# zhengchen1999/DOVE

Measured on AMD Instinct MI355X. Metric: SR frames/s (33x720x1280 4x one-step, whole job), higher is better.
Workload: dtype bf16; 1 GPU; synthetic 33x720x1280 HR clip (LR 180x320, 4x), one-step t=399, CogVideoX1.5-5B VAE + 42-layer DiT random-init, 1 clip per GPU (BASELINE configs[1]); weight_sums=True, vae_streams=2, variant=headline (bf16)

## Files before the change

### dove_amd/csrc/elementwise.hip

```cpp
#include "common.h"
#include "../../include/dove_hip.h"

__device__ __forceinline__ float load_any(const void* p, long long i, int dt) {
  return dt == DOVE_F32 ? ((const float*)p)[i] : bf2f(((const bf16_t*)p)[i]);
}
__device__ __forceinline__ void store_any(void* p, long long i, int dt, float v) {
  if (dt == DOVE_F32) ((float*)p)[i] = v;
  else ((bf16_t*)p)[i] = f2bf(v);
}

__global__ void cl_from_ncthw_kernel(const void* __restrict__ x, int dt, int C, long long npix, int Cp,
                                     float scale, float shift, bf16_t* __restrict__ y) {
  const long long p = (long long)blockIdx.x * blockDim.x + threadIdx.x;
  if (p >= npix) return;
  bf16_t* yr = y + p * Cp;
  for (int c0 = 0; c0 < Cp; c0 += 8) {
    float f[8];
#pragma unroll
    for (int e = 0; e < 8; ++e) {
      const int c = c0 + e;
      f[e] = c < C ? load_any(x, (long long)c * npix + p, dt) * scale + shift : 0.f;
    }
    *(uint4*)(yr + c0) = pack8(f);
  }
}

extern "C" int dove_cl_from_ncthw(const void* x, int dtype, int C, long long npix, int Cp, float scale, float shift,
                                   void* y, void* stream) {
  DOVE_CHECK_ARG(x && y, "cl_from_ncthw: null pointer");
  DOVE_CHECK_ARG(dtype == DOVE_F32 || dtype == DOVE_BF16, "cl_from_ncthw: bad dtype %d", dtype);
  DOVE_CHECK_ARG(Cp % 8 == 0 && Cp >= C && C > 0 && npix > 0, "cl_from_ncthw: need Cp %% 8 == 0, Cp >= C");
  hipLaunchKernelGGL(cl_from_ncthw_kernel, dim3((unsigned)((npix + 255) / 256)), dim3(256), 0, (hipStream_t)stream, x,
                     dtype, C, npix, Cp, scale, shift, (bf16_t*)y);
  DOVE_CHECK_LAUNCH("dove_cl_from_ncthw");
  return DOVE_OK;
}

__global__ void cl_im2col3x3_kernel(const void* __restrict__ x, int dt, int C, int T, int H, int W, int Cp, float scale, float shift,
                                    bf16_t* __restrict__ y) {
  const long long npix = (long long)T * H * W;
  const long long p = (long long)blockIdx.x * blockDim.x + threadIdx.x;
  if (p >= npix) return;
  const int w = (int)(p % W), h = (int)((p / W) % H);
  bf16_t* yr = y + p * Cp;
  for (int c0 = 0; c0 < Cp; c0 += 8) {
    float f[8];
#pragma unroll
    for (int e = 0; e < 8; ++e) {
      const int k = c0 + e, tap = k / C, c = k - tap * C;
      const int dy = tap / 3 - 1, dx = tap % 3 - 1;
      const bool in = tap < 9 && h + dy >= 0 && h + dy < H && w + dx >= 0 && w + dx < W;
      f[e] = in ? load_any(x, (long long)c * npix + p + (long long)dy * W + dx, dt) * scale + shift : 0.f;
    }
    *(uint4*)(yr + c0) = pack8(f);
  }
}
extern "C" int dove_cl_im2col3x3_from_ncthw(const void* x, int dtype, int C, int T, int H, int W, int Cp, float scale, float shift, void* y,
                                            void* stream) {
  DOVE_CHECK_ARG(x && y, "cl_im2col3x3: null pointer");
  DOVE_CHECK_ARG(dtype == DOVE_F32 || dtype == DOVE_BF16, "cl_im2col3x3: bad dtype %d", dtype);
  DOVE_CHECK_ARG(C > 0 && Cp % 8 == 0 && Cp >= 9 * C && T > 0 && H > 0 && W > 0, "cl_im2col3x3: need Cp %% 8 == 0 and Cp >= 9 C");
  const long long npix = (long long)T * H * W;
  hipLaunchKernelGGL(cl_im2col3x3_kernel, dim3((unsigned)((npix + 255) / 256)), dim3(256), 0, (hipStream_t)stream, x, dtype, C, T, H, W, Cp,
                     scale, shift, (bf16_t*)y);
  DOVE_CHECK_LAUNCH("dove_cl_im2col3x3_from_ncthw");
  return DOVE_OK;
}

__global__ void ncthw_from_cl_kernel(const bf16_t* __restrict__ x, long long ld, int C, long long npix, float scale,
                                     float shift, float lo, float hi, void* __restrict__ y, int dt) {
  const long long p = (long long)blockIdx.x * blockDim.x + threadIdx.x;
  if (p >= npix) return;
  const bf16_t* xr = x + p * ld;
  for (int c0 = 0; c0 < C; c0 += 4) {
    const uint2 v = *(const uint2*)(xr + c0);
    const float f[4] = {__uint_as_float(v.x << 16), __uint_as_float(v.x & 0xffff0000u), __uint_as_float(v.y << 16),
                        __uint_as_float(v.y & 0xffff0000u)};
#pragma unroll
    for (int e = 0; e < 4; ++e)
      if (c0 + e < C) store_any(y, (long long)(c0 + e) * npix + p, dt, fminf(fmaxf(f[e] * scale + shift, lo), hi));
  }
}

extern "C" int dove_ncthw_from_cl(const void* x, long long ld, int C, long long npix, float scale, float shift,
                                   float lo, float hi, void* y, int dtype, void* stream) {
  DOVE_CHECK_ARG(x && y, "ncthw_from_cl: null pointer");
  DOVE_CHECK_ARG(dtype == DOVE_F32 || dtype == DOVE_BF16, "ncthw_from_cl: bad dtype %d", dtype);
  DOVE_CHECK_ARG(ld % 4 == 0 && ld >= ((C + 3) / 4) * 4 && C > 0 && npix > 0, "ncthw_from_cl: ld must be a multiple of 4 covering C");
  hipLaunchKernelGGL(ncthw_from_cl_kernel, dim3((unsigned)((npix + 255) / 256)), dim3(256), 0, (hipStream_t)stream,
                     (const bf16_t*)x, ld, C, npix, scale, shift, lo, hi, y, dtype);
  DOVE_CHECK_LAUNCH("dove_ncthw_from_cl");
  return DOVE_OK;
}

__global__ __launch_bounds__(256) void conv_out_gather_kernel(const float* __restrict__ p, int ldp, int T, int H, int W, int C,
                                                              const float* __restrict__ bias, float scale, float shift, float lo, float hi,
                                                              void* __restrict__ y, int dt, int ldy) {
  extern __shared__ __attribute__((aligned(16))) float tile[];
  constexpr int TH = 8, TW = 64, RW = TW + 2, NREC = (TH + 2) * RW;
  const int lrec = ldp + 1, f4n = ldp >> 2;
  const int x0 = blockIdx.x * TW, y0 = blockIdx.y * TH, t = blockIdx.z;
  for (int i = threadIdx.x; i < NREC * f4n; i += 256) {
    const int rec = i / f4n, f4 = i - rec * f4n;
    const int ry = rec / RW, rx = rec - ry * RW;
    const int iy = y0 + ry - 1, ix = x0 + rx - 1;
    f32x4 v = {0.f, 0.f, 0.f, 0.f};
    if (iy >= 0 && iy < H && ix >= 0 && ix < W) v = *(const f32x4*)(p + (((long long)t * H + iy) * W + ix) * ldp + f4 * 4);
    float* d = tile + rec * lrec + f4 * 4;
    d[0] = v[0]; d[1] = v[1]; d[2] = v[2]; d[3] = v[3];
  }
  __syncthreads();
  const int lx = threadIdx.x & 63;
  const long long npix = (long long)T * H * W;
#pragma unroll
  for (int h2 = 0; h2 < 2; ++h2) {
    const int rr = (threadIdx.x >> 6) + 4 * h2;
// ... 354 lines not shown
```

### dove_amd/csrc/igemm.hip

```cpp
#include "igemm_args.h"


template <int BN, int BK>
struct FastCfg {
  static constexpr int BM = 128;
  static constexpr int CPR = BK / 8;
  static constexpr int CPR_LOG = (BK == 64) ? 3 : 2;
  static constexpr int RPG = 256 / CPR;
  static constexpr int NA = BM / RPG;
  static constexpr int B_SLOTS = BN * CPR;
  static constexpr int NB = (B_SLOTS + 255) / 256;
  static constexpr int A_BYTES = BM * BK * 2, B_BYTES = BN * BK * 2, STAGE = A_BYTES + B_BYTES;
  static constexpr int WN = (BN >= 128) ? 2 : 1, WM = 4 / WN;
  static constexpr int PT = (BM / WM) / 32, CT = (BN / WN) / 32;
  static constexpr int KK = BK / 16;
};

template <int BN, int BK>
__global__ __launch_bounds__(256) void igemm_fast_kernel(const IgemmArgs a) {
  using Cf = FastCfg<BN, BK>;
  constexpr int NA = Cf::NA, NB = Cf::NB, PT = Cf::PT, CT = Cf::CT, KK = Cf::KK, STAGE = Cf::STAGE, A_BYTES = Cf::A_BYTES;
  extern __shared__ __attribute__((aligned(16))) char smem[];
  const int tid = threadIdx.x, lane = tid & 63;
  const int wave = __builtin_amdgcn_readfirstlane(tid >> 6);
// ... 1023 lines not shown
namespace smallk { constexpr int ROWS = 32; }
__global__ __launch_bounds__(256) void smallk_kernel(const bf16_t* __restrict__ x, const bf16_t* __restrict__ w, const float* __restrict__ bias,
                                                     bf16_t* __restrict__ out, long long M, int cout_store, long long ldo) {
  typedef __bf16 v2bf __attribute__((ext_vector_type(2)));
  __shared__ uint4 xs[4 * smallk::ROWS][4];
  const int lane = threadIdx.x & 63, wave = threadIdx.x >> 6;
  const long long rb = (long long)blockIdx.x * 4 * smallk::ROWS;
#pragma unroll
  for (int i = 0; i < 2; ++i) {
    const int idx = threadIdx.x + i * 256;
    const long long m = rb + (idx >> 2);
    xs[idx >> 2][idx & 3] = m < M ? *(const uint4*)(x + m * 32 + (idx & 3) * 8) : uint4{0u, 0u, 0u, 0u};
  }
  const int n0 = (blockIdx.y * 64 + lane) * 4;
  const bool live = n0 < cout_store;
  uint32_t wr[4][16];
  float b[4] = {0.f, 0.f, 0.f, 0.f};
  if (live) {
#pragma unroll
    for (int j = 0; j < 4; ++j)
#pragma unroll
      for (int q = 0; q < 4; ++q) {
        const uint4 v = *(const uint4*)(w + (long long)(n0 + j) * 32 + q * 8);
        wr[j][q * 4 + 0] = v.x; wr[j][q * 4 + 1] = v.y; wr[j][q * 4 + 2] = v.z; wr[j][q * 4 + 3] = v.w;
      }
    if (bias) { b[0] = bias[n0]; b[1] = bias[n0 + 1]; b[2] = bias[n0 + 2]; b[3] = bias[n0 + 3]; }
  }
  __syncthreads();
  if (!live) return;
  const long long r0 = rb + wave * smallk::ROWS;
#pragma unroll 4
  for (int r = 0; r < smallk::ROWS; ++r) {
    const long long m = r0 + r;
    if (m >= M) break;
    uint32_t xr[16];
#pragma unroll
    for (int q = 0; q < 4; ++q) {
      const uint4 v = xs[wave * smallk::ROWS + r][q];
      xr[q * 4 + 0] = v.x; xr[q * 4 + 1] = v.y; xr[q * 4 + 2] = v.z; xr[q * 4 + 3] = v.w;
    }
    float acc[4] = {b[0], b[1], b[2], b[3]};
#pragma unroll
    for (int k = 0; k < 16; ++k)
#pragma unroll
      for (int j = 0; j < 4; ++j)
        acc[j] = __builtin_amdgcn_fdot2_f32_bf16(__builtin_bit_cast(v2bf, wr[j][k]), __builtin_bit_cast(v2bf, xr[k]), acc[j], false);
    uint2 o;
    o.x = pack_bf2(acc[0], acc[1]);
    o.y = pack_bf2(acc[2], acc[3]);
    *(uint2*)(out + m * ldo + n0) = o;
  }
}

enum ConvKernel { K_IGEMM = 0, K_IGEMM_FAST, K_HALO4X, K_HALO4X_UP, K_GEMM8P, K_SMALLK, K_HALO4X_SUB };
static const char* const kKernelNames[] = {"igemm_kernel", "igemm_fast_kernel", "conv3x3_halo4x_kernel", "conv3x3_halo4x_kernel", "gemm8p_kernel",
                                           "smallk_kernel", "conv3x3_halo4x_kernel"};

static inline int desc_nb(const dove_conv_desc* d) { return d->nb > 1 ? d->nb : 1; }

static ConvKernel select_kernel(const dove_conv_desc* d) {
  const long long M = (long long)desc_nb(d) * d->t_out * d->h_out * d->w_out;
  const bool frame_fits = (long long)d->h_in * d->w_in * d->cin * 2 < (1ll << 31);
  const bool plain_gemm = d->kt == 1 && d->kh == 1 && d->kw == 1 && d->stride == 1 && d->up == 0 && d->tmode == 0 &&
                          d->t_in == d->t_out && d->h_in == d->h_out && d->w_in == d->w_out && d->cout_pad % 128 == 0 && M >= 4096 &&
                          (long long)512 * d->cin * 2 < (1ll << 31);
  const bool pointwise = d->kt == 1 && d->kh == 1 && d->kw == 1 && d->stride == 1 && d->up == 0 && d->tmode == 0 && d->t_in == d->t_out &&
                         d->h_in == d->h_out && d->w_in == d->w_out;
  if (pointwise && d->cin == 32 && d->act == 0 && !d->resid && !d->gate && d->cout_store >= 128) return K_SMALLK;
  if (plain_gemm) {
    if (d->cout_pad % 256 == 0 && d->cout_store % 256 == 0 && d->cin % 128 == 0 && d->cin >= 256 && (long long)256 * d->cin * 2 < (1ll << 31) &&
        d->ldo < (1 << 20) && d->ldr < (1 << 20) && (d->act == 0 || d->act == 1))
      return K_GEMM8P;
  }
  const bool conv3 = d->kh == 3 && d->kw == 3 && d->stride == 1 && d->pad_h == 1 && d->pad_w == 1 && d->act == 0 && !d->gate &&
                     d->cout_pad % 128 == 0 && frame_fits;
  if (conv3) {
    const bool same = d->up == 0 && d->tmode == 0 && d->h_out == d->h_in && d->w_out == d->w_in && d->w_out >= 16 && d->h_out >= 16;
    const bool ups = d->up == 1 && d->kt == 1 && d->h_out == 2 * d->h_in && d->w_out == 2 * d->w_in && d->h_out >= 16 && d->w_out >= 32;
    const bool h4 = d->cout_store % 128 == 0 && d->cin % 64 == 0 && d->ldo < (1 << 20) && (!d->resid || d->ldr < (1 << 20));
    if (same && h4) return K_HALO4X;
    if (ups && h4 && d->w_sub && d->h_in >= 16 && d->w_in >= 32) return K_HALO4X_SUB;
    if (ups && h4) return K_HALO4X_UP;
  }
  const int BN = (d->cout_pad % 128 == 0) ? 128 : ((d->cout_pad % 64 == 0) ? 64 : 32);
  const bool fits = frame_fits && (long long)BN * d->cin * 2 < (1ll << 31);
  return (d->up == 0 && fits) ? K_IGEMM_FAST : K_IGEMM;
}

static bool desc_size_ok(const dove_conv_desc* d, const char* who) {
  if (d && d->struct_size == sizeof(dove_conv_desc) && d->reserved == 0) return true;
  if (d) dove_set_error("%s: dove_conv_desc.struct_size is %u, this library (ABI %d) expects %zu - the caller's binding was written "
                        "against another include/dove_hip.h", who, d->struct_size, DOVE_ABI_VERSION, sizeof(dove_conv_desc));
  else dove_set_error("%s: null descriptor", who);
  return false;
}
extern "C" const char* dove_conv_kernel_name(const dove_conv_desc* d) { return desc_size_ok(d, "conv_kernel_name") ? kKernelNames[select_kernel(d)] : ""; }

template <int BN, int BK>
static int launch_igemm_fast(const IgemmArgs& a, unsigned grid, hipStream_t s) {
  constexpr int lds = 2 * (128 * BK * 2 + BN * BK * 2);
  static PerDeviceOnce attr_set;
  if (auto once_ = attr_set.guard()) (void)hipFuncSetAttribute((const void*)igemm_fast_kernel<BN, BK>, hipFuncAttributeMaxDynamicSharedMemorySize, lds);
  hipLaunchKernelGGL((igemm_fast_kernel<BN, BK>), dim3(grid), dim3(256), lds, s, a);
  DOVE_CHECK_LAUNCH("dove_conv_igemm_bf16");
  return DOVE_OK;
}

static int cu_count() {
  static std::atomic<int> cus[DOVE_MAX_DEVICES] = {};
  int dev = 0;
  (void)hipGetDevice(&dev);
  int n = (dev >= 0 && dev < DOVE_MAX_DEVICES) ? cus[dev].load(std::memory_order_relaxed) : 0;
  if (!n) {
    n = 256;
    (void)hipDeviceGetAttribute(&n, hipDeviceAttributeMultiprocessorCount, dev);
    if (dev >= 0 && dev < DOVE_MAX_DEVICES) cus[dev].store(n, std::memory_order_relaxed);
  }
  return n;
}

extern "C" long long dove_conv_gn_partial_rows(const dove_conv_desc* d) {
  if (!desc_size_ok(d, "conv_gn_partial_rows")) return 0;
  const ConvKernel k = select_kernel(d);
  if (k != K_HALO4X && k != K_HALO4X_UP && k != K_HALO4X_SUB) return 0;
  if (d->cout_store != 128 && d->cout_store != 256 && d->cout_store != 512) return 0;
  if (d->cout_store != d->cout_pad) return 0;
  if (k == K_HALO4X_SUB) {
    const long long th = (d->h_in + halo8::TH - 1) / halo8::TH, tw = (d->w_in + halo8::TW - 1) / halo8::TW;
    return (long long)desc_nb(d) * d->t_out * th * tw * 16;
  }
  const long long th = (d->h_out + halo8::TH - 1) / halo8::TH, tw = (d->w_out + halo8::TW - 1) / halo8::TW;
  return (long long)desc_nb(d) * d->t_out * th * tw * 4;
}

static bool halo4x_plan(const dove_conv_desc* d) {
  const int tiles_w = (d->w_out + halo8::TW - 1) / halo8::TW, tiles_h = (d->h_out + halo8::TH - 1) / halo8::TH;
  const int wrem = d->w_out % halo8::TW;
  if (wrem < 1 || wrem > halo8::TW / 2) return false;
  const int cus = cu_count();
  const long long per = (long long)desc_nb(d) * d->t_out * (d->cout_pad / 128);
  auto rounds = [&](long long tiles) { return (tiles * per + cus - 1) / cus; };
  return rounds((long long)tiles_h * (tiles_w - 1)) + rounds((d->h_out + 31) / 32) < rounds((long long)tiles_h * tiles_w);
}
extern "C" int dove_conv_partial_launches(const dove_conv_desc* d) {
  if (!desc_size_ok(d, "conv_partial_launches") || select_kernel(d) != K_HALO4X) return 0;
  return halo4x_plan(d) ? 1 : 0;
}

static int conv_dispatch(const dove_conv_desc* d, void* stream, ConvKernel kern);

static bool gemm_tail_split(const dove_conv_desc* d, long long* rows_main) {
  const long long M = (long long)d->t_out * d->h_out * d->w_out;
  if (d->t_out != 1 || d->h_out != 1 || desc_nb(d) > 1) return false;
  const int cus = cu_count(), tiles_n = d->cout_pad / 256;
  const long long row_tiles = (M + gemm4x::BM - 1) / gemm4x::BM, ntiles = row_tiles * tiles_n;
  if (ntiles <= cus || ntiles % cus == 0) return false;
  const long long main_rt = (ntiles / cus) * cus / tiles_n;
// ... 110 lines not shown
      a.tiles_n = 4 * (d->cout_pad / 128);
      a.nty = a.tiles_h; a.ntx = a.tiles_w; a.h_lim = d->h_out; a.w_lim = d->w_out;
      const long long g4 = (long long)a.T_out * a.tiles_h * a.tiles_w * a.tiles_n;
      DOVE_CHECK_ARG(g4 > 0 && g4 < (1ll << 31), "conv_igemm: grid too large");
      static PerDeviceOnce attrs;
      if (auto once_ = attrs.guard()) (void)hipFuncSetAttribute((const void*)(conv3x3_halo4x_kernel<false, true>), hipFuncAttributeMaxDynamicSharedMemorySize, Halo4xCfg::LDS_BYTES);
      const int cus = cu_count();
      const unsigned grid = g4 > cus ? (unsigned)cus : (unsigned)g4;
      hipLaunchKernelGGL((conv3x3_halo4x_kernel<false, true>), dim3(grid), dim3(256), Halo4xCfg::LDS_BYTES, s, a);
      DOVE_CHECK_LAUNCH("dove_conv_igemm_bf16(halo4x sub-pixel)");
      return DOVE_OK;
    }
    case K_HALO4X:
    case K_HALO4X_UP: {
      a.gn_partial = d->gn_partial;
      a.w_first = (kern == K_HALO4X && d->kt == 3 && !d->cache) ? (const bf16_t*)d->w_first : nullptr;
      if (kern == K_HALO4X && d->kt == 3 && d->tdup) { a.tdup = d->tdup; a.w_pair = (const bf16_t*)d->w_pair; }
      a.cpg_log = d->cout_store == 128 ? 2 : (d->cout_store == 256 ? 3 : 4);
      a.tiles_w = (d->w_out + halo8::TW - 1) / halo8::TW;
      a.tiles_h = (d->h_out + halo8::TH - 1) / halo8::TH;
      a.tiles_n = d->cout_pad / 128;
      a.ty0 = a.tx0 = 0; a.nty = a.tiles_h; a.ntx = a.tiles_w; a.h_lim = d->h_out; a.w_lim = d->w_out;
      const long long g4 = (long long)a.T_out * a.tiles_h * a.tiles_w * a.tiles_n;
      DOVE_CHECK_ARG(g4 > 0 && g4 < (1ll << 31), "conv_igemm: grid too large");
      static PerDeviceOnce attr4;
      if (auto once_ = attr4.guard()) {
        (void)hipFuncSetAttribute((const void*)(conv3x3_halo4x_kernel<false>), hipFuncAttributeMaxDynamicSharedMemorySize, Halo4xCfg::LDS_BYTES);
        (void)hipFuncSetAttribute((const void*)(conv3x3_halo4x_kernel<false, false, 1>), hipFuncAttributeMaxDynamicSharedMemorySize, H4Geo<1>::LDS_BYTES);
        (void)hipFuncSetAttribute((const void*)(conv3x3_halo4x_kernel<true>), hipFuncAttributeMaxDynamicSharedMemorySize, Halo4xCfg::LDS_BYTES);
      }
      const int cus = cu_count();
      const unsigned grid = g4 > cus ? (unsigned)cus : (unsigned)g4;
      if (kern == K_HALO4X_UP) hipLaunchKernelGGL((conv3x3_halo4x_kernel<true>), dim3(grid), dim3(256), Halo4xCfg::LDS_BYTES, s, a);
      else {
        const bool wpart = halo4x_plan(d);
        const int wm = wpart ? (a.tiles_w - 1) * halo8::TW : d->w_out, cols_main = wpart ? a.tiles_w - 1 : a.tiles_w;
        auto launch = [&](int part, int nty, int tx0, int ntx, int w_lim) {
          if (nty <= 0 || ntx <= 0) return;
          IgemmArgs b = a;
          b.ty0 = 0; b.nty = nty; b.tx0 = tx0; b.ntx = ntx; b.h_lim = d->h_out; b.w_lim = w_lim;
          const long long g = (long long)b.T_out * nty * ntx * b.tiles_n;
          const unsigned gr = g > cus ? (unsigned)cus : (unsigned)g;
          if (part == 0) hipLaunchKernelGGL((conv3x3_halo4x_kernel<false, false, 0>), dim3(gr), dim3(256), H4Geo<0>::LDS_BYTES, s, b);
          else hipLaunchKernelGGL((conv3x3_halo4x_kernel<false, false, 1>), dim3(gr), dim3(256), H4Geo<1>::LDS_BYTES, s, b);
        };
        launch(0, a.tiles_h, 0, cols_main, wm);
        if (wpart) launch(1, (d->h_out + 31) / 32, cols_main, 1, d->w_out);
      }
      DOVE_CHECK_LAUNCH("dove_conv_igemm_bf16(halo4x)");
      return DOVE_OK;
    }
    default: break;
  }
  int twl = 7;
  if (d->h_out > 1) {
    twl = 4;
    if (d->w_out <= 8) twl = 3;
    if (d->w_out <= 4) twl = 2;
  }
  a.tw_log2 = twl;
  const int TW = 1 << twl, TH = 128 >> twl;
  a.tiles_w = (d->w_out + TW - 1) / TW;
  a.tiles_h = (d->h_out + TH - 1) / TH;
  const int BN = (d->cout_pad % 128 == 0) ? 128 : ((d->cout_pad % 64 == 0) ? 64 : 32);
  a.tiles_n = d->cout_pad / BN;
  const long long grid = (long long)a.T_out * a.tiles_h * a.tiles_w * a.tiles_n;
  DOVE_CHECK_ARG(grid > 0 && grid < (1ll << 31), "conv_igemm: grid too large");
  const bool fast = kern == K_IGEMM_FAST;
  const bool bk64 = (d->cin % 64 == 0);
  if (!fast) return launch_igemm_legacy(a, (unsigned)grid, BN, bk64, s);
  if (BN == 128) return bk64 ? launch_igemm_fast<128, 64>(a, (unsigned)grid, s) : launch_igemm_fast<128, 32>(a, (unsigned)grid, s);
  if (BN == 64) return bk64 ? launch_igemm_fast<64, 64>(a, (unsigned)grid, s) : launch_igemm_fast<64, 32>(a, (unsigned)grid, s);
  return bk64 ? launch_igemm_fast<32, 64>(a, (unsigned)grid, s) : launch_igemm_fast<32, 32>(a, (unsigned)grid, s);
}
```

### dove_amd/lib.py

```python
from __future__ import annotations

import ctypes as C
import os

import torch

_HERE = os.path.dirname(os.path.abspath(__file__))
LIB_PATH = os.path.join(_HERE, "libdove_hip.so")
_lib = None

F32, BF16, U8 = 0, 1, 2
METRIC_PSNR, METRIC_SSIM, METRIC_RGB_TO_Y = 1, 2, 4
COLORFIX_WAVELET, COLORFIX_ADAIN, COLORFIX_CLAMP = 1, 2, 1
YUV_444, YUV_422, YUV_420, YUV_MONO = 0, 1, 2, 3
YUV_SITING_LEFT, YUV_SITING_CENTRE = 0, 1
VIDEO_RGB_U8, VIDEO_YUV = 0, 1
RESIZE_BILINEAR, RESIZE_BICUBIC, RESIZE_AREA = 0, 1, 2
ACT_NONE, ACT_RELU, ACT_SIGMOID, ACT_TANH = 0, 1, 2, 3


class ConvDesc(C.Structure):
    _fields_ = [
        ("struct_size", C.c_uint), ("reserved", C.c_uint),
        ("x", C.c_void_p), ("cache", C.c_void_p), ("w", C.c_void_p), ("bias", C.c_void_p),
# ... 147 lines not shown
    "dove_linear_mxfp8": [_VP, _VP, _VP, _VP, _VP, _VP, _VP, _VP, _LL, _I, _I, _LL, _LL, _LL, _I, _VP],
    "dove_fr_metrics": [C.POINTER(ImageView), C.POINTER(ImageView), _I, _I, _I, _I, _I, _VP, C.c_size_t, _VP, _VP],
    "dove_color_fix": [C.POINTER(ImageView), _F, _F, C.POINTER(ImageView), _F, _F, _I, _I, _I, _I, _I, C.POINTER(ImageView), _VP,
                       C.c_size_t, _VP],
    "dove_rgb_to_yuv_u8": [C.POINTER(ImageView), _I, _I, _I, C.POINTER(YuvFormat), _VP, _VP],
    "dove_yuv_to_rgb_u8": [_VP, _I, _I, _I, C.POINTER(YuvFormat), _VP, _VP],
    "dove_plan_padding": [_I, _I, _I, _PI, _PI, _PI],
    "dove_plan_output_size": [_I, _I, _I, _PI, _PI],
    "dove_plan_temporal_chunks": [_I, _I, _I, _PI, _I],
    "dove_plan_spatial_tiles": [_I, _I, _I, _I, _I, _I, _PI, _I],
    "dove_plan_valid_region": [_PI, _I, _I, _I, _I, _I, _I, _PI, _PI],
    "dove_plan_pieces": [_I, _I, _I, _I, _I, _I, _I, _I, _I, _PI, _PI, _PI, _I],
    "dove_plan_check_coverage": [_PI, _I, _I, _I, _I],
    "dove_chunk_planner_create": [_I, _I, C.POINTER(_VP)],
    "dove_chunk_planner_next": [_VP, _LL, _I, _PLL, _PLL, _PI],
    "dove_philox_u32": [_VP, _LL, _ULL, _ULL, _ULL, _VP],
    "dove_randn": [_VP, _I, _LL, _ULL, _ULL, _ULL, _VP],
    "dove_blur2d_f32": [_VP, _I, _I, _I, _VP, _I, _I, _VP, _VP],
    "dove_resize_f32": [_VP, _I, _I, _I, _I, _I, _I, _VP, _VP],
    "dove_add_gaussian_noise_f32": [_VP, _I, _I, _I, C.POINTER(C.c_float), _I, _ULL, _ULL, _LL, _VP, _VP],
    "dove_add_poisson_noise_f32": [_VP, _I, _I, _I, C.POINTER(C.c_float), _I, _ULL, _ULL, _LL, _VP, C.c_size_t, _VP, _VP],
    "dove_jpeg_roundtrip": [_VP, _I, _I, _I, _PI, _VP, C.c_size_t, _VP, _VP],
    "dove_stitch": [_VP, _I, _I, _I, _PI, _VP, _I, _I, _I, _I, _I, _I, _VP],
    "dove_video_open": [_VP, C.POINTER(VideoParams), C.POINTER(_VP)],
    "dove_video_info": [_VP, C.POINTER(C.c_size_t), C.POINTER(C.c_size_t), _PI, _PI, _PI],
    "dove_video_push": [_VP, _VP, _I, _VP],
    "dove_video_end_of_input": [_VP],
    "dove_video_need": [_VP, _PLL, _PI],
    "dove_video_step": [_VP, _VP, C.c_size_t, _PI, _PI, _VP],
    "dove_conv2d_f32": [C.POINTER(Conv2dF32Args), _VP],
    "dove_instance_norm_f32": [_VP, _I, _I, _I, _I, _VP, _I, _F, _VP, C.c_size_t, _VP, _VP],
    "dove_corr_volume_f32": [_VP, _VP, _I, _I, _I, _I, _F, _VP, _VP],
    "dove_avgpool2_f32": [_VP, _LL, _I, _I, _VP, _VP],
    "dove_corr_lookup_f32": [_VP, _VP, _VP, _VP, _VP, _LL, _I, _I, _I, _I, _VP, _VP],
    "dove_gru_gate_f32": [_VP, _LL, _VP, _LL, _I, _I, _LL, _VP, _VP],
    "dove_gru_update_f32": [_VP, _LL, _VP, _LL, _VP, _LL, _I, _LL, _VP],
    "dove_add_f32": [_VP, _LL, _VP, _LL, _VP, _LL, _I, _LL, _I, _VP],
    "dove_convex_upsample_f32": [_VP, _LL, _VP, _I, _I, _I, _VP, _VP],
    "dove_flow_warp_error": [_VP, _VP, _I, _VP, _VP, _I, _I, _I, _VP, C.c_size_t, _VP, _VP, _VP, _VP],
    "dove_convnet_conv_f32": [C.POINTER(ConvnetConvF32Args), _VP],
    "dove_percep_prep_f32": [C.POINTER(ImageView), _I, _I, _I, _I, _F, _F, C.POINTER(C.c_float), C.POINTER(C.c_float), _VP, _VP],
    "dove_maxpool_f32": [_VP, _LL, _I, _I, _I, _I, _I, _I, _VP, _LL, _VP],
    "dove_l2pool_f32": [_VP, _LL, _I, _I, _I, _I, _VP, _LL, _VP],
    "dove_lpips_layer": [_VP, _VP, _LL, _VP, _I, _I, _I, _I, _VP, C.c_size_t, _VP, _VP],
    "dove_dists_layer": [_VP, _VP, _LL, _VP, _VP, _I, _I, _I, _I, _VP, C.c_size_t, _VP, _VP],
    "dove_niqe_features": [C.POINTER(ImageView), _I, _I, _I, _I, _VP, C.c_size_t, _VP, _VP, _VP],
    "dove_niqe_stats": [_VP, _I, _I, _VP, _VP, _VP, _VP],
    "dove_niqe_distance": [_VP, _VP, _VP, _VP, _VP],
}
PLAIN = {"dove_last_error": (C.c_char_p, []), "dove_abi_version": (C.c_int, []), "dove_comm_destroy": (None, [C.c_void_p]),
         "dove_conv_gn_partial_rows": (C.c_longlong, [C.POINTER(ConvDesc)]),
         "dove_conv_kernel_name": (C.c_char_p, [C.POINTER(ConvDesc)]),
         "dove_conv_partial_launches": (C.c_int, [C.POINTER(ConvDesc)]),
         "dove_attention_head_paths": (C.c_int, [C.POINTER(C.c_float), _I, C.POINTER(C.c_int)]),
         "dove_attention_path_name": (C.c_char_p, [_I]),
         "dove_device_info": (C.c_int, [_I, C.c_char_p, _I, C.POINTER(C.c_int), C.POINTER(C.c_longlong)]),
         "dove_destroy": (None, [_VP]),
         "dove_vae_decode_num_frames": (C.c_int, [_VP, _I]),
         "dove_get_option": (C.c_longlong, [_VP, _I]),
         "dove_comm_useful_ranks": (C.c_int, [_VP, _I, _I]),
         "dove_workspace_bytes": (C.c_size_t, [_VP, _I, _I, _I]),
         "dove_workspace_high_water": (C.c_size_t, [_VP]),
         "dove_fr_metrics_workspace_bytes": (C.c_size_t, [_I, _I, _I]),
         "dove_color_fix_workspace_bytes": (C.c_size_t, [_I, _I, _I, _I]),
         "dove_yuv_frame_bytes": (C.c_size_t, [_I, _I, _I]),
         "dove_poisson_noise_workspace_bytes": (C.c_size_t, [_I]),
         "dove_jpeg_roundtrip_workspace_bytes": (C.c_size_t, [_I, _I, _I]),
         "dove_chunk_planner_need": (C.c_longlong, [_VP]),
         "dove_chunk_planner_destroy": (None, [_VP]),
         "dove_video_workspace_bytes": (C.c_size_t, [_VP, C.POINTER(VideoParams)]),
         "dove_video_close": (None, [_VP]),
         "dove_instance_norm_f32_workspace_bytes": (C.c_size_t, [_I, _I, _I, _I]),
         "dove_flow_warp_error_workspace_bytes": (C.c_size_t, [_I, _I, _I]),
         "dove_convnet_conv_f32_kernel_name": (C.c_char_p, [C.POINTER(ConvnetConvF32Args)]),
         "dove_lpips_layer_workspace_bytes": (C.c_size_t, [_I, _I, _I]),
         "dove_dists_layer_workspace_bytes": (C.c_size_t, [_I, _I, _I, _I]),
         "dove_niqe_workspace_bytes": (C.c_size_t, [_I, _I, _I])}


def kernel_source_sha256() -> str:
    import glob
    import hashlib
    h = hashlib.sha256()
    files = sorted(glob.glob(os.path.join(_HERE, "csrc", "*.hip")) + glob.glob(os.path.join(_HERE, "csrc", "*.h")))
    files.append(os.path.join(os.path.dirname(_HERE), "include", "dove_hip.h"))
    for fn in files:
        h.update(os.path.basename(fn).encode() + b"\0")
        with open(fn, "rb") as f:
            h.update(f.read())
        h.update(b"\0")
    return h.hexdigest()


def load():
    global _lib
    if _lib is not None:
        return _lib
    if not os.path.exists(LIB_PATH):
        raise RuntimeError(f"{LIB_PATH} not found: build it with `python -c 'import __graft_entry__ as g; g.build()'` "
                           "(dove_amd has no CPU fallback)")
    lib = C.CDLL(LIB_PATH)
    for name, argt in SIGNATURES.items():
        fn = getattr(lib, name)
        fn.argtypes = argt
        fn.restype = C.c_int
    for name, (res, argt) in PLAIN.items():
# ... 42 lines not shown
```

### include/dove_hip.h

```cpp
#ifndef DOVE_HIP_H
#define DOVE_HIP_H

#include <stddef.h>

#ifdef __cplusplus
extern "C" {
#endif

#define DOVE_ABI_VERSION 15

#define DOVE_F32 0
#define DOVE_BF16 1

const char* dove_last_error(void);
int dove_abi_version(void);
int dove_device_info(int dev, char* name, int name_len, int* cu_count, long long* total_mem);

typedef struct dove_conv_desc {
  unsigned int struct_size;
  unsigned int reserved;
  const void* x;
  const void* cache;
  const void* w;
  const float* bias;
  const void* resid;
  const float* gate;
  void* out;
  int t_in, h_in, w_in, cin;
  int t_out, h_out, w_out, cout_pad, cout_store;
  int kt, kh, kw, stride, pad_h, pad_w, up, tmode, act;
  long long ldo, ldr, gate_split;
  float* gn_partial;
  int out_f32;
  int nb;
  long long cache_stride;
  const void* w_first;
  const void* w_sub;
  const void* w_pair;
  int tdup;
  int reserved2;
} dove_conv_desc;
int dove_conv_igemm_bf16(const dove_conv_desc* d, void* stream);
const char* dove_conv_kernel_name(const dove_conv_desc* d);
int dove_conv_partial_launches(const dove_conv_desc* d);
long long dove_conv_gn_partial_rows(const dove_conv_desc* d);
int dove_groupnorm_finalize_partials(const float* partial, long long rows, double count, float eps, void* ws, float* stats,
                                     void* stream);

int dove_groupnorm_stats_bf16(const void* x, long long npix, long long frame_pix, int C, float eps, void* partial_ws, int ws_blocks,
                              float* stats, void* stream);
int dove_groupnorm_sums_bf16(const void* x, long long npix, long long frame_pix, int C, void* partial_ws, int ws_blocks, double* sums,
                             void* stream);
int dove_groupnorm_finalize_sums(const double* sums, double count, float eps, float* stats, void* stream);
int dove_groupnorm_sums_from_partials(const float* partial, long long rows, void* ws, double* sums, void* stream);
int dove_groupnorm_apply_bf16(const void* x, void* y, int T, int H, int W, int C, const float* stats,
                              const float* gamma, const float* beta, int silu, const void* yb, int hz, int wz,
                              int sshift, const int* tmap, void* stream);

int dove_groupnorm_stats_nb_bf16(const void* x, int nb, long long npix, long long frame_pix, int C, float eps, void* partial_ws,
                                 int ws_blocks, float* stats, void* stream);
int dove_groupnorm_finalize_partials_nb(const float* partial, long long rows, int nb, double count, float eps, void* ws, size_t ws_bytes,
                                        float* stats, void* stream);
int dove_groupnorm_apply_nb_bf16(const void* x, void* y, int nb, int T, int H, int W, int C, const float* stats, const float* gamma,
                                 const float* beta, int silu, const void* yb, int Tz, int hz, int wz, int sshift, const int* tmap,
                                 void* stream);
int dove_avgpool_time_nb_bf16(const void* x, int nb, int T, long long frame_elems, void* y, void* stream);

int dove_layernorm_modulate_bf16(const void* x, void* y, long long rows, int D, float eps, const float* gamma,
                                 const float* beta, const float* mod, long long split, void* stream);

int dove_qkv_post_bf16(const void* qkv, long long N, long long Npad, int heads, int head_dim, int text_len,
                       const float* gq, const float* bq, const float* gk, const float* bk, const float* cosT,
                       const float* sinT, float qscale, float eps, void* Qh, void* Kh, void* Vt, int v_order, float* norm2, void* stream);
int dove_vt_quad_swap_bf16(void* Vt, long long rows, long long Npad, void* stream);
int dove_ulysses_place_bf16(const void* rq, const void* rk, const void* rv, const long long* counts, int world, int hloc, long long N,
                            long long Npad, void* Qh, void* Kh, void* Vt, float* norm2_out, void* stream);

int dove_attention_fwd_bf16(const void* Qh, const void* Kh, const void* Vt, void* O, long long N, long long Npad,
                            int heads, int head_dim, long long ldo, float* norm2, void* stream);
int dove_attention_head_paths(const float* norm2_host, int heads, int* path);
const char* dove_attention_path_name(int path);

int dove_cl_from_ncthw(const void* x, int dtype, int C, long long npix, int Cp, float scale, float shift, void* y,
                       void* stream);
int dove_ncthw_from_cl(const void* x, long long ld, int C, long long npix, float scale, float shift, float lo,
                       float hi, void* y, int dtype, void* stream);
int dove_cl_im2col3x3_from_ncthw(const void* x, int dtype, int C, int T, int H, int W, int Cp, float scale, float shift, void* y,
                                 void* stream);
int dove_conv_out_gather(const float* p, long long ldp, int T, int H, int W, int C, const float* bias, float scale, float shift, float lo,
                         float hi, void* y, int dtype, void* stream);
int dove_avgpool_time_bf16(const void* x, int T, long long frame_elems, void* y, void* stream);
int dove_posterior_sample(const void* moments, long long ld, int latent_channels, long long npix, const void* noise,
                          int noise_dtype, void* out, int out_dtype, void* stream);
int dove_axpby(const void* x, const void* y, void* out, int dtype, long long n, float a, float b, void* stream);
int dove_patchify(const void* x, int dtype, int T, int C, int H, int W, int pt, int p, void* tokens, long long ld,
                  void* stream);
int dove_unpatchify(const void* tokens, long long ld, int T, int C, int H, int W, int pt, int p, void* y, int dtype,
// ... 255 lines not shown
```

Measured before the change: 35.54 frames/s.

## Add persistent thin-K pointwise conv kernel with LDS-resident weights

Adds a persistent igemm_thin kernel for pointwise convs with small K (64–384) and narrow Cout (32/128/256). It keeps all weights resident in LDS and streams activation tiles through a per-wave ring with counted vmcnt waits, then writes output through an LDS epilogue with buffer stores. The aim is to avoid reloading weights for every tile and the poor tile shapes of the generic fast igemm on these thin GEMMs. Separately, the 3x3 im2col kernel now uses one thread per 8-channel chunk instead of one per pixel, with 32-bit index math when it fits, giving more parallelism and cheaper addressing. The price is a much larger, more complex kernel with a grid limited to one block per CU, and correctness depends on the hand-counted waits.

```diff
diff --git a/dove_amd/csrc/elementwise.hip b/dove_amd/csrc/elementwise.hip
--- a/dove_amd/csrc/elementwise.hip
+++ b/dove_amd/csrc/elementwise.hip
@@ -36,32 +36,41 @@
   return DOVE_OK;
 }
 
+template <typename I>
+__device__ __forceinline__ void cl_im2col3x3_chunk(const void* __restrict__ x, int dt, int C, I npix, int H, int W, int Cp, float scale, float shift,
+                                                   bf16_t* __restrict__ y, I i) {
+  const I cpp = (I)(Cp >> 3);
+  const I p = i / cpp;
+  if (p >= npix) return;
+  const int c0 = (int)(i - p * cpp) << 3;
+  const I row = p / (I)W;
+  const int w = (int)(p - row * (I)W), h = (int)(row % (I)H);
+  int tap = c0 / C, c = c0 - tap * C;
+  float f[8];
+#pragma unroll
+  for (int e = 0; e < 8; ++e) {
+    const int ty = tap / 3, dy = ty - 1, dx = tap - ty * 3 - 1;
+    const bool in = tap < 9 && h + dy >= 0 && h + dy < H && w + dx >= 0 && w + dx < W;
+    f[e] = in ? load_any(x, (long long)c * (long long)npix + (long long)p + (long long)(dy * W + dx), dt) * scale + shift : 0.f;
+    if (++c == C) { c = 0; ++tap; }
+  }
+  *(uint4*)(y + (long long)p * Cp + c0) = pack8(f);
+}
 __global__ void cl_im2col3x3_kernel(const void* __restrict__ x, int dt, int C, int T, int H, int W, int Cp, float scale, float shift,
                                     bf16_t* __restrict__ y) {
   const long long npix = (long long)T * H * W;
-  const long long p = (long long)blockIdx.x * blockDim.x + threadIdx.x;
-  if (p >= npix) return;
-  const int w = (int)(p % W), h = (int)((p / W) % H);
-  bf16_t* yr = y + p * Cp;
-  for (int c0 = 0; c0 < Cp; c0 += 8) {
-    float f[8];
-#pragma unroll
-    for (int e = 0; e < 8; ++e) {
-      const int k = c0 + e, tap = k / C, c = k - tap * C;
-      const int dy = tap / 3 - 1, dx = tap % 3 - 1;
-      const bool in = tap < 9 && h + dy >= 0 && h + dy < H && w + dx >= 0 && w + dx < W;
-      f[e] = in ? load_any(x, (long long)c * npix + p + (long long)dy * W + dx, dt) * scale + shift : 0.f;
-    }
-    *(uint4*)(yr + c0) = pack8(f);
-  }
+  const long long i = (long long)blockIdx.x * blockDim.x + threadIdx.x;
+  if (npix * (Cp >> 3) + 256 < (1ll << 32)) cl_im2col3x3_chunk<unsigned>(x, dt, C, (unsigned)npix, H, W, Cp, scale, shift, y, (unsigned)i);
+  else cl_im2col3x3_chunk<long long>(x, dt, C, npix, H, W, Cp, scale, shift, y, i);
 }
 extern "C" int dove_cl_im2col3x3_from_ncthw(const void* x, int dtype, int C, int T, int H, int W, int Cp, float scale, float shift, void* y,
                                             void* stream) {
   DOVE_CHECK_ARG(x && y, "cl_im2col3x3: null pointer");
   DOVE_CHECK_ARG(dtype == DOVE_F32 || dtype == DOVE_BF16, "cl_im2col3x3: bad dtype %d", dtype);
   DOVE_CHECK_ARG(C > 0 && Cp % 8 == 0 && Cp >= 9 * C && T > 0 && H > 0 && W > 0, "cl_im2col3x3: need Cp %% 8 == 0 and Cp >= 9 C");
-  const long long npix = (long long)T * H * W;
-  hipLaunchKernelGGL(cl_im2col3x3_kernel, dim3((unsigned)((npix + 255) / 256)), dim3(256), 0, (hipStream_t)stream, x, dtype, C, T, H, W, Cp,
+  const long long nchunk = (long long)T * H * W * (Cp / 8);
+  DOVE_CHECK_ARG((nchunk + 255) / 256 < (1ll << 31), "cl_im2col3x3: grid too large");
+  hipLaunchKernelGGL(cl_im2col3x3_kernel, dim3((unsigned)((nchunk + 255) / 256)), dim3(256), 0, (hipStream_t)stream, x, dtype, C, T, H, W, Cp,
                      scale, shift, (bf16_t*)y);
   DOVE_CHECK_LAUNCH("dove_cl_im2col3x3_from_ncthw");
   return DOVE_OK;
diff --git a/dove_amd/csrc/igemm.hip b/dove_amd/csrc/igemm.hip
--- a/dove_amd/csrc/igemm.hip
+++ b/dove_amd/csrc/igemm.hip
@@ -1099,6 +1099,203 @@
   }
 }
 
+template <int BK, int COUT, bool F32>
+struct ThinCfg {
+  static constexpr int R = 4;
+  static constexpr int CPR = BK / 8;
+  static constexpr int SLOT = 32 * BK * 2;
+  static constexpr int NL = SLOT / 1024;
+  static constexpr int NT = COUT / 32;
+  static constexpr int KK = BK / 16;
+  static constexpr int ESZ = F32 ? 4 : 2;
+  static constexpr int PC = F32 ? 32 : (COUT < 64 ? COUT : 64);
+  static constexpr int TPP = PC / 32, NP = COUT / PC;
+  static constexpr int EROWB = PC * ESZ, EPITCH = EROWB + 16;
+  static constexpr int ESLICE = 32 * EPITCH;
+  static constexpr int LPR = EROWB / 16, RPS = 64 / LPR;
+  static constexpr int NSP = 32 / RPS, NS = NP * NSP;
+  static constexpr int WSTEP = COUT * BK * 2;
+  static constexpr int IPS = WSTEP / 1024;
+  static constexpr int lds_bytes(int nk) { return nk * WSTEP + COUT * 4 + 4 * R * SLOT + 4 * ESLICE; }
+  static_assert((R - 1) * NL + 2 * NS < 64, "counted waits must fit vmcnt's 6 bits");
+};
+__device__ __forceinline__ const bf16_t* thin_pin64(const bf16_t* p) {
+  const unsigned long long v = (unsigned long long)p;
+  return (const bf16_t*)(((unsigned long long)(unsigned)__builtin_amdgcn_readfirstlane((int)(v >> 32)) << 32) |
+                         (unsigned)__builtin_amdgcn_readfirstlane((int)v));
+}
+__device__ __forceinline__ int thin_tile_frame(unsigned lg, int tpf, int T, int kt) {
+  return __builtin_amdgcn_readfirstlane(kt > 1 ? (int)(lg % (unsigned)T) : (int)(lg / (unsigned)tpf));
+}
+__device__ __forceinline__ int thin_tile_hw0(unsigned lg, int t, int tpf, int T, int kt) {
+  return __builtin_amdgcn_readfirstlane((kt > 1 ? (int)(lg / (unsigned)T) : (int)(lg - (unsigned)t * (unsigned)tpf)) << 7);
+}
+template <int N> __device__ __forceinline__ void thin_wait_vm() { asm volatile("s_waitcnt vmcnt(%0)" ::"n"(N) : "memory"); }
+
+template <int BK, int COUT, bool F32>
+__global__ __launch_bounds__(256, 1) void igemm_thin_kernel(const IgemmArgs a) {
+#if defined(__HIP_DEVICE_COMPILE__)
+  using Cf = ThinCfg<BK, COUT, F32>;
+  constexpr int R = Cf::R, NL = Cf::NL, NT = Cf::NT, KK = Cf::KK, NS = Cf::NS, SLOT = Cf::SLOT, ESZ = Cf::ESZ;
+  extern __shared__ __attribute__((aligned(16))) char smem[];
+  const int tid = threadIdx.x, lane = tid & 63;
+  const int wave = __builtin_amdgcn_readfirstlane(tid >> 6);
+  __builtin_assume(wave >= 0 && wave < 4);
+  const int hi = lane >> 5, l31 = lane & 31;
+
+  const int kcp = a.Cin / BK, nk = a.kt * kcp;
+  const int HW = a.H_out * a.W_out;
+  const int tpf = (HW + 127) >> 7;
+  const int ntiles = a.T_out * tpf, G = (int)gridDim.x;
+  const long long frame_elems = (long long)HW * a.Cin;
+  char* const wlds = smem;
+  float* const bias_l = (float*)(smem + nk * Cf::WSTEP);
+  char* const ring = smem + nk * Cf::WSTEP + COUT * 4 + wave * (R * SLOT);
+  char* const esl = smem + nk * Cf::WSTEP + COUT * 4 + 4 * R * SLOT + wave * Cf::ESLICE;
+
+  auto swz = [](int row) { return BK == 64 ? ((row >> 1) & 7) : ((row >> 2) & 3); };
+  unsigned voffA[NL];
+#pragma unroll
+  for (int j = 0; j < NL; ++j) {
+    const int q = j * 64 + lane, row = q / Cf::CPR, cs = q % Cf::CPR;
+    voffA[j] = (unsigned)((row * a.Cin + ((cs ^ swz(row)) << 3)) * 2);
+  }
+  int xoff[KK];
+#pragma unroll
+  for (int kk = 0; kk < KK; ++kk) xoff[kk] = l31 * (BK * 2) + (((kk * 2 + hi) ^ swz(l31)) << 4);
+
+  if (tid < COUT) bias_l[tid] = (a.bias && tid < a.Cout_st) ? a.bias[tid] : 0.f;
+  asm volatile("s_waitcnt vmcnt(0)" ::: "memory");
+  {
+    const auto srd_w = __builtin_amdgcn_make_buffer_rsrc((void*)a.w, (short)0, (int)((long long)a.kt * a.Cout_pad * a.Cin * 2), 0x00020000);
+    const int wq = lane / Cf::CPR, wcs = lane % Cf::CPR;
+    for (int idx = wave; idx < nk * Cf::IPS; idx += 4) {
+      const int s = idx / Cf::IPS, q = idx - s * Cf::IPS;
+      const int tap = s / kcp, kc = s - tap * kcp;
+      const int row = q * (64 / Cf::CPR) + wq;
+      const unsigned voff = (unsigned)((((tap * a.Cout_pad + row) * a.Cin) + kc * BK + ((wcs ^ swz(row)) << 3)) * 2);
+      __builtin_amdgcn_raw_ptr_buffer_load_lds(srd_w, (lds_ptr_t)(wlds + idx * 1024), 16, voff, 0, 0, 0);
+    }
+  }
+
+  int n_id = 0, n_t = 0, n_hw0 = 0, n_vw = 0, n_dt = 0, n_kc = 0;
+  bool n_on = false;
+  auto open_tile = [&](int id) {
+    n_id = id;
+    n_on = id < ntiles;
+    const unsigned lg = xcd_remap((unsigned)(n_on ? id : ntiles - 1), (unsigned)ntiles);
+    n_t = thin_tile_frame(lg, tpf, a.T_out, a.kt);
+    n_hw0 = thin_tile_hw0(lg, n_t, tpf, a.T_out, a.kt);
+    const int left = HW - n_hw0 - wave * 32;
+    n_vw = __builtin_amdgcn_readfirstlane(left < 0 ? 0 : (left > 32 ? 32 : left));
+    n_dt = 0; n_kc = 0;
+  };
+  auto stage_next = [&](int slot) {
+    const bf16_t* fp = thin_pin64(igemm_src_frame(a, n_t, n_dt, frame_elems));
+    const bf16_t* src = fp + (long long)(n_hw0 + wave * 32) * a.Cin + n_kc * BK;
+    const int nrec0 = n_on ? n_vw * a.Cin * 2 - n_kc * (BK * 2) : 0;
+    const int nrec = __builtin_amdgcn_readfirstlane(nrec0 > 0 ? nrec0 : 0);
+    const auto srd = __builtin_amdgcn_make_buffer_rsrc((void*)thin_pin64(src), (short)0, nrec, 0x00020000);
+#pragma unroll
+    for (int j = 0; j < NL; ++j)
+      __builtin_amdgcn_raw_ptr_buffer_load_lds(srd, (lds_ptr_t)(ring + slot * SLOT + j * 1024), 16, voffA[j], 0, 0, 0);
+    if (++n_kc == kcp) {
+      n_kc = 0;
+      if (++n_dt == a.kt) open_tile(n_id + G);
+    }
+  };
+  open_tile((int)blockIdx.x);
+#pragma unroll
+  for (int r = 0; r < R; ++r) stage_next(r);
+  thin_wait_vm<R * NL>();
+  asm volatile("s_waitcnt lgkmcnt(0)" ::: "memory");
+  __builtin_amdgcn_s_barrier();
+  asm volatile("" ::: "memory");
+
+  const int e_row = lane / Cf::LPR, e_ch = lane % Cf::LPR;
+  const unsigned esl_w = (unsigned)(size_t)(__attribute__((address_space(3))) char*)esl + l31 * Cf::EPITCH;
+
+  int g = 0;
+  int ep1 = -2 * R, ep2 = -2 * R;
+  for (int id = (int)blockIdx.x; id < ntiles; id += G) {
+    f32x16 acc[NT];
+#pragma unroll
+    for (int i = 0; i < NT; ++i)
+#pragma unroll
+      for (int r = 0; r < 16; ++r) acc[i][r] = 0.f;
+
+    for (int s = 0; s < nk; ++s, ++g) {
+      const int e = (ep1 >= g - R ? 1 : 0) + (ep2 >= g - R ? 1 : 0);
+      if (e == 0) thin_wait_vm<(R - 1) * NL>();
+      else if (e == 1) thin_wait_vm<(R - 1) * NL + NS>();
+      else thin_wait_vm<(R - 1) * NL + 2 * NS>();
+      const int slot = g & (R - 1);
+      const char* xs = ring + slot * SLOT;
+      const char* ws = wlds + s * Cf::WSTEP;
+      bf16x8 xf[KK], wf[KK][NT];
+#pragma unroll
+      for (int kk = 0; kk < KK; ++kk) {
+        xf[kk] = *(const bf16x8*)(xs + xoff[kk]);
+#pragma unroll
+        for (int i = 0; i < NT; ++i) wf[kk][i] = *(const bf16x8*)(ws + i * (32 * BK * 2) + xoff[kk]);
+      }
+#pragma unroll
+      for (int kk = 0; kk < KK; ++kk)
+#pragma unroll
+        for (int i = 0; i < NT; ++i) acc[i] = __builtin_amdgcn_mfma_f32_32x32x16_bf16(wf[kk][i], xf[kk], acc[i], 0, 0, 0);
+      asm volatile("s_waitcnt lgkmcnt(0)" ::: "memory");
+      stage_next(slot);
+    }
+
+    {
+      const unsigned lg = xcd_remap((unsigned)id, (unsigned)ntiles);
+      const int t = thin_tile_frame(lg, tpf, a.T_out, a.kt);
+      const int hw0 = thin_tile_hw0(lg, t, tpf, a.T_out, a.kt);
+      const int left = HW - hw0 - wave * 32;
+      const int vw = left < 0 ? 0 : (left > 32 ? 32 : left);
+      const long long pix0 = (long long)t * HW + hw0 + wave * 32;
+      const int rowb = (int)a.ldo * ESZ;
+      const auto srd_o = __builtin_amdgcn_make_buffer_rsrc((void*)thin_pin64((const bf16_t*)((char*)a.out + pix0 * a.ldo * ESZ)), (short)0,
+                                                           __builtin_amdgcn_readfirstlane(vw * rowb), 0x00020000);
+#pragma unroll
+      for (int p = 0; p < Cf::NP; ++p) {
+#pragma unroll
+        for (int ti = 0; ti < Cf::TPP; ++ti) {
+          const int i = p * Cf::TPP + ti;
+#pragma unroll
+          for (int q = 0; q < 4; ++q) {
+            const int cl = ti * 32 + 8 * q + 4 * hi;
+            const f32x4 b = *(const f32x4*)(bias_l + p * Cf::PC + cl);
+            const f32x4 v = {acc[i][q * 4 + 0] + b[0], acc[i][q * 4 + 1] + b[1], acc[i][q * 4 + 2] + b[2], acc[i][q * 4 + 3] + b[3]};
+            if (F32) asm volatile("ds_write_b128 %0, %1" ::"v"(esl_w + cl * 4), "v"(v) : "memory");
+            else {
+              const unsigned long long pk = (unsigned long long)pack_bf2(v[0], v[1]) | ((unsigned long long)pack_bf2(v[2], v[3]) << 32);
+              asm volatile("ds_write_b64 %0, %1" ::"v"(esl_w + cl * 2), "v"(pk) : "memory");
+            }
+          }
+        }
+        asm volatile("s_waitcnt lgkmcnt(0)" ::: "memory");
+        u32x4 o[Cf::NSP];
+#pragma unroll
+        for (int j = 0; j < Cf::NSP; ++j) o[j] = *(const u32x4*)(esl + (j * Cf::RPS + e_row) * Cf::EPITCH + e_ch * 16);
+        asm volatile("s_waitcnt lgkmcnt(0)" ::: "memory");
+        const bool chv = p * Cf::PC + (e_ch + 1) * (16 / ESZ) <= a.Cout_st;
+#pragma unroll
+        for (int j = 0; j < Cf::NSP; ++j) {
+          const unsigned off = chv ? (unsigned)((j * Cf::RPS + e_row) * rowb + e_ch * 16) : 0x80000000u;
+          __builtin_amdgcn_raw_buffer_store_b128(o[j], srd_o, (int)off, p * Cf::EROWB, 0);
+          __builtin_amdgcn_sched_barrier(0);
+          asm volatile("s_nop 3" ::: "memory");
+          __builtin_amdgcn_sched_barrier(0);
+        }
+      }
+    }
+    ep2 = ep1; ep1 = g - 1;
+  }
+  asm volatile("s_waitcnt vmcnt(0)" ::: "memory");
+#endif
+}
+
 enum ConvKernel { K_IGEMM = 0, K_IGEMM_FAST, K_HALO4X, K_HALO4X_UP, K_GEMM8P, K_SMALLK, K_HALO4X_SUB };
 static const char* const kKernelNames[] = {"igemm_kernel", "igemm_fast_kernel", "conv3x3_halo4x_kernel", "conv3x3_halo4x_kernel", "gemm8p_kernel",
                                            "smallk_kernel", "conv3x3_halo4x_kernel"};
@@ -1150,6 +1347,34 @@
   if (auto once_ = attr_set.guard()) (void)hipFuncSetAttribute((const void*)igemm_fast_kernel<BN, BK>, hipFuncAttributeMaxDynamicSharedMemorySize, lds);
   hipLaunchKernelGGL((igemm_fast_kernel<BN, BK>), dim3(grid), dim3(256), lds, s, a);
   DOVE_CHECK_LAUNCH("dove_conv_igemm_bf16");
+  return DOVE_OK;
+}
+
+static bool thin_walk_ok(const dove_conv_desc* d) {
+  const int K = d->kt * d->cin, esz = d->out_f32 ? 4 : 2;
+  const bool shape = d->kh == 1 && d->kw == 1 && d->stride == 1 && d->up == 0 && d->tmode == 0 && d->pad_h == 0 && d->pad_w == 0 &&
+                     d->t_in == d->t_out && d->h_in == d->h_out && d->w_in == d->w_out && !d->gate && d->act == 0 && !d->resid;
+  if (!shape || K > 384 || K < 64) return false;
+  if (d->cout_pad != 32 && d->cout_pad != 128 && d->cout_pad != 256) return false;
+  if ((long long)K * d->cout_pad * 2 > 96 * 1024) return false;
+  if (d->out_f32 && d->cout_pad == 256) return false;
+  if (d->cout_store % (16 / esz) != 0 || (d->ldo * esz) % 16 != 0 || ((uintptr_t)d->out & 15) != 0 || d->ldo >= (1 << 22)) return false;
+  if ((long long)d->h_out * d->w_out >= (1ll << 24)) return false;
+  return true;
+}
+extern "C" int dove_conv_thin_walk(const dove_conv_desc* d) {
+  return desc_size_ok(d, "conv_thin_walk") && select_kernel(d) == K_IGEMM_FAST && thin_walk_ok(d) ? 1 : 0;
+}
+
+template <int BK, int COUT, bool F32>
+static int launch_igemm_thin(const IgemmArgs& a, unsigned grid, hipStream_t s) {
+  using Cf = ThinCfg<BK, COUT, F32>;
+  const int lds = Cf::lds_bytes(a.kt * (a.Cin / BK));
+  static PerDeviceOnce attr_set;
+  if (auto once_ = attr_set.guard())
+    (void)hipFuncSetAttribute((const void*)igemm_thin_kernel<BK, COUT, F32>, hipFuncAttributeMaxDynamicSharedMemorySize, 160 * 1024);
+  hipLaunchKernelGGL((igemm_thin_kernel<BK, COUT, F32>), dim3(grid), dim3(256), lds, s, a);
+  DOVE_CHECK_LAUNCH("dove_conv_igemm_bf16(thin)");
   return DOVE_OK;
 }
 
@@ -1366,6 +1591,22 @@
     }
     default: break;
   }
+  if (kern == K_IGEMM_FAST && thin_walk_ok(d)) {
+    const long long tpf = ((long long)d->h_out * d->w_out + 127) / 128, nt = (long long)a.T_out * tpf;
+    DOVE_CHECK_ARG(nt > 0 && nt < (1ll << 31), "conv_igemm: grid too large");
+    a.tw_log2 = 7; a.tiles_w = (int)tpf; a.tiles_h = 1; a.tiles_n = 1;
+    const int cus = cu_count();
+    const unsigned grid = nt > cus ? (unsigned)cus : (unsigned)nt;
+    const bool k64 = d->cin % 64 == 0 && (long long)d->kt * d->cin * d->cout_pad * 2 <= 64 * 1024;
+    const bool f32 = d->out_f32 != 0;
+#define DOVE_THIN(COUT)                                                                                                   \
+  return k64 ? (f32 ? launch_igemm_thin<64, COUT, true>(a, grid, s) : launch_igemm_thin<64, COUT, false>(a, grid, s))   \
+             : (f32 ? launch_igemm_thin<32, COUT, true>(a, grid, s) : launch_igemm_thin<32, COUT, false>(a, grid, s))
+    if (d->cout_pad == 32) { DOVE_THIN(32); }
+    if (d->cout_pad == 128) { DOVE_THIN(128); }
+#undef DOVE_THIN
+    return k64 ? launch_igemm_thin<64, 256, false>(a, grid, s) : launch_igemm_thin<32, 256, false>(a, grid, s);
+  }
   int twl = 7;
   if (d->h_out > 1) {
     twl = 4;
diff --git a/dove_amd/lib.py b/dove_amd/lib.py
--- a/dove_amd/lib.py
+++ b/dove_amd/lib.py
@@ -223,6 +223,7 @@
          "dove_conv_gn_partial_rows": (C.c_longlong, [C.POINTER(ConvDesc)]),
          "dove_conv_kernel_name": (C.c_char_p, [C.POINTER(ConvDesc)]),
          "dove_conv_partial_launches": (C.c_int, [C.POINTER(ConvDesc)]),
+         "dove_conv_thin_walk": (C.c_int, [C.POINTER(ConvDesc)]),
          "dove_attention_head_paths": (C.c_int, [C.POINTER(C.c_float), _I, C.POINTER(C.c_int)]),
          "dove_attention_path_name": (C.c_char_p, [_I]),
          "dove_device_info": (C.c_int, [_I, C.c_char_p, _I, C.POINTER(C.c_int), C.POINTER(C.c_longlong)]),
diff --git a/include/dove_hip.h b/include/dove_hip.h
--- a/include/dove_hip.h
+++ b/include/dove_hip.h
@@ -43,6 +43,7 @@
 int dove_conv_igemm_bf16(const dove_conv_desc* d, void* stream);
 const char* dove_conv_kernel_name(const dove_conv_desc* d);
 int dove_conv_partial_launches(const dove_conv_desc* d);
+int dove_conv_thin_walk(const dove_conv_desc* d);
 long long dove_conv_gn_partial_rows(const dove_conv_desc* d);
 int dove_groupnorm_finalize_partials(const float* partial, long long rows, double count, float eps, void* ws, float* stats,
                                      void* stream);
```

Measured after the change: 35.79 frames/s (median of 6 runs). Within noise of the previous version (+0.7%).
